# PABannier/biogpt.cpp

Measured on AMD Instinct MI355X. Metric: decode tokens/sec BioGPT Q4_0 n_ctx=1024, higher is better.
Workload: dtype int8; 1 GPU; greedy 200-token continuation of a 4-token prompt per GPU (main.cpp loop, -b 8, --top_k 1), BioGPT-base Q4_0, F32 KV cache, n_ctx=1024; 1 step = 1 continuation per rank; n_layer=24, d_model=1024, d_ff=4096, n_vocab=42384, n_predict=200, n_prompt=4, parallelism=replicas x1 (weights RCCL-broadcast once)

## Files before the change

biogpt.cpp_amd/csrc/kernels_xpipe.hip.h:

```cpp
#pragma once

#include "kernels_decode.hip.h"

namespace bgk {

typedef unsigned long long xp_u64;
typedef float xp_v4f __attribute__((ext_vector_type(4)));
#define XP_RLX __ATOMIC_RELAXED, __HIP_MEMORY_SCOPE_AGENT
constexpr uint32_t XP_SPIN_MAX = 400000u;

struct XpLayer {
    const float *ln0_w, *ln0_b, *ln1_w, *ln1_b;
    const float *bqkv, *bo, *b1, *b2;
    DevMatrix Wqkv, Wo, W1, W2;
    float *kcache, *vcache;
    unsigned long long *gx1, *gx;
};

constexpr int XP_G_QKV = 0;
constexpr int XP_G_ATT = 3072;
constexpr int XP_G_X1 = XP_G_ATT + 320;
constexpr int XP_G_H = XP_G_X1 + 1024;
constexpr int XP_G_X = XP_G_H + 1280;
constexpr int XP_G_LAYER = XP_G_X + 1024;
// ... 234 lines not shown
    for (int r = 16; r < 64; r += 16) {
        const float ov = __int_as_float(__builtin_amdgcn_readlane(__float_as_int(bv), r));
        const int oi = __builtin_amdgcn_readlane(bi, r);
        if (ov > rv || (ov == rv && oi < ri)) { rv = ov; ri = oi; }
    }
    bv = rv; bi = ri;
}
template <int WT>
__device__ __forceinline__ void xp_row4_request(const DevMatrix &m, int row, int t, uint32_t &q, uint32_t &sc, uint32_t &qh) {
    using TI = TypeInfo<WT>;
    const int64_t blk = (int64_t)row * (m.K / QK) + (t >> 3);
    const int j = (4 * t) & 31;
    if (WT == W_Q8_0) q = *reinterpret_cast<const uint32_t *>(m.qs + blk * 32 + j);
    else q = *reinterpret_cast<const uint32_t *>(m.qs + blk * 16 + (j & 15));
    sc = TI::q81 ? reinterpret_cast<const uint32_t *>(m.sc)[blk] : (uint32_t)reinterpret_cast<const uint16_t *>(m.sc)[blk];
    qh = (WT == W_Q5_0 || WT == W_Q5_1) ? m.qh[blk] : 0u;
}
template <int WT>
__device__ __forceinline__ void xp_row4_values(uint32_t q, uint32_t sc, uint32_t qh, int t, float (&e)[4]) {
    const int j = (4 * t) & 31;
#pragma unroll
    for (int i = 0; i < 4; i++) {
        if (WT == W_Q8_0) { e[i] = __fmul_rn((float)(int8_t)((q >> (8 * i)) & 0xFFu), h2f((uint16_t)sc)); continue; }
        const uint32_t byte = (q >> (8 * i)) & 0xFFu;
        int v = (j < 16) ? (int)(byte & 0x0Fu) : (int)(byte >> 4);
        if (WT == W_Q5_0 || WT == W_Q5_1) v |= (int)((qh >> (j + i)) & 1u) << 4;
        if (WT == W_Q4_0) e[i] = __fmul_rn((float)(v - 8), h2f((uint16_t)sc));
        else if (WT == W_Q5_0) e[i] = __fmul_rn((float)(v - 16), h2f((uint16_t)sc));
        else e[i] = __fadd_rn(__fmul_rn((float)v, h2f((uint16_t)(sc & 0xFFFFu))), h2f((uint16_t)(sc >> 16)));
    }
}

__device__ __forceinline__ uint32_t xp_pack4(int8_t q) {
    const int b = (int)(uint8_t)q;
    const int b1 = __builtin_amdgcn_update_dpp(0, b, 0x101, 0xf, 0xf, true);
    const int b2 = __builtin_amdgcn_update_dpp(0, b, 0x102, 0xf, 0xf, true);
    const int b3 = __builtin_amdgcn_update_dpp(0, b, 0x103, 0xf, 0xf, true);
    return (uint32_t)b | ((uint32_t)b1 << 8) | ((uint32_t)b2 << 16) | ((uint32_t)b3 << 24);
}

constexpr int XL_G_SC = 0;
constexpr int XL_G_PV = 16 * 1024;
constexpr int XL_G_LAYER = XL_G_PV + 16 * 16 * 128;

constexpr int XP_S_X = 0;
constexpr int XP_S_X1 = XP_S_X + 4096;
constexpr int XP_S_XQ = XP_S_X1 + 4096;
constexpr int XP_S_XD = XP_S_XQ + 1024;
constexpr int XP_S_XS = XP_S_XD + 128;
constexpr int XP_S_RED = XP_S_XS + 128;
constexpr int XP_S_HQ = XP_S_RED + 64;
constexpr int XP_S_HD = XP_S_HQ + 4096;
constexpr int XP_S_HS = XP_S_HD + 512;
constexpr int XP_S_PART = XP_S_HS + 512;
constexpr int XP_S_G = XP_S_PART + 256 * DEC_PS * 4;
constexpr int XP_S_LN = XP_S_G + 512;
constexpr int XP_S_BIAS = XP_S_LN + 16384;
constexpr int XP_S_CUR = XP_S_BIAS + 1536;
constexpr int XP_S_S = XP_S_CUR + 768;
constexpr int XP_S_REDF = XP_S_S + 1024;
constexpr int XP_S_REDD = XP_S_REDF + 512;
constexpr int XP_S_PV = XP_S_REDD + 128;
constexpr int XP_S_TOTAL = XP_S_PV + 8192;
static_assert(32 * DEC_PS2 <= 256 * DEC_PS, "fc2 block terms fit the shared region");
__host__ __device__ inline size_t xpipe_smem_bytes(int gelu_entries) { return XP_S_TOTAL + (size_t)gelu_entries * 2; }

template <int WT, bool EXPAND>
__device__ __forceinline__ float xp_dot(const Unit<WT> &u, const uint32_t *xq, float xd, float xs_f, int xs_i) {
    if constexpr (EXPAND) return unit_dot_settled<WT>(u, xq, xd, xs_f, xs_i);
    else return unit_dot_quant<WT>(u, xq, xd, xs_f, xs_i);
}
template <int WT, bool EXPAND>
__device__ __forceinline__ void xp_settle(Unit<WT> &u) {
    if constexpr (EXPAND) {
        settle_unit<WT>(u);
        asm volatile("" : "+v"(u.q0.x), "+v"(u.q0.y), "+v"(u.q0.z), "+v"(u.q0.w), "+v"(u.q1.x), "+v"(u.q1.y), "+v"(u.q1.z), "+v"(u.q1.w), "+v"(u.sc));
    }
}

__device__ __forceinline__ uint32_t xp_wave_sum_u32(uint32_t v) {
    int s = (int)v;
    s += dpp_i<DPP_QUAD_XOR1>(s); s += dpp_i<DPP_QUAD_XOR2>(s); s += dpp_i<DPP_ROW_HALF_MIRROR>(s); s += dpp_i<DPP_ROW_MIRROR>(s);
    return (uint32_t)((__builtin_amdgcn_readlane(s, 0) + __builtin_amdgcn_readlane(s, 16)) + (__builtin_amdgcn_readlane(s, 32) + __builtin_amdgcn_readlane(s, 48)));
}

template <int WT, int LPK, int NW, int KCAP, int ROLE, bool SPLIT, bool RES>
__device__ __forceinline__ void xp_run(const XpParams &p, unsigned char *smem, const int xcd, const int slot, const uint32_t epoch0, const int n_past0,
                                       const int n_gen0) {
    using TI = TypeInfo<WT>;
    static_assert(TI::quant && (WT != W_Q8_0 || SPLIT), "18-30 weight units per lane must fit the register file (Q8_0: 9 registers per unit: split layers)");
    static_assert(ROLE == 0 || ROLE == 1 || (ROLE == 2 && SPLIT), "0 attention head, 1 q/k/v rows, 2 (split layers) the MLP half");
    static_assert(SPLIT || TI::q81, "the producers publish Q8_0 block sums only for Q4_1 / Q5_1 (want_sum = q81): the symmetric formats need the signed units of the split form (unit_dot_settled)");
    constexpr bool ATTN = ROLE == 0;
    constexpr bool EXPAND = SPLIT;
    constexpr bool FIRST = !SPLIT || ROLE != 2, SECOND = !SPLIT || ROLE == 2;
    static_assert(LPK == 2 || LPK == 4 || LPK == 8 || LPK == 16, "lanes per key");
    static_assert(NW == 8 || NW == 16, "waves per workgroup");
    constexpr int D = 1024, DK = 64, NT = NW * 64;
    constexpr int QS = 96 / NW, OS = 16 / NW, FS = 64 / NW, F2R = 32 / NW;
    constexpr bool DUAL = SPLIT && KCAP > 256;
    constexpr int KW = DUAL ? KCAP / 2 : KCAP;
    constexpr int HI = (DUAL && ROLE == 1) ? 1 : 0;
    static_assert(KW % NW == 0 && KW <= NW * 64 / LPK, "key capacity of the launch");
    constexpr int NF4 = 16 / LPK, NV = KW / NW;
    float *const s_x = reinterpret_cast<float *>(smem + XP_S_X);
    float *const s_x1 = reinterpret_cast<float *>(smem + XP_S_X1);
    uint32_t *const s_xq = reinterpret_cast<uint32_t *>(smem + XP_S_XQ);
    float *const s_xd = reinterpret_cast<float *>(smem + XP_S_XD);
    uint32_t *const s_xs = reinterpret_cast<uint32_t *>(smem + XP_S_XS);
    double *const s_red = reinterpret_cast<double *>(smem + XP_S_RED);
    uint32_t *const s_hq = reinterpret_cast<uint32_t *>(smem + XP_S_HQ);
    float *const s_hd = reinterpret_cast<float *>(smem + XP_S_HD);
    uint32_t *const s_hs = reinterpret_cast<uint32_t *>(smem + XP_S_HS);
    float *const s_part = reinterpret_cast<float *>(smem + XP_S_PART);
    float *const s_g = reinterpret_cast<float *>(smem + XP_S_G);
    float *const s_ln = reinterpret_cast<float *>(smem + XP_S_LN);
    float *const s_bias = reinterpret_cast<float *>(smem + XP_S_BIAS);
    float *const s_cur = reinterpret_cast<float *>(smem + XP_S_CUR);
    float *const s_S = reinterpret_cast<float *>(smem + XP_S_S);
    float *const s_redf = reinterpret_cast<float *>(smem + XP_S_REDF);
    int *const s_redi = reinterpret_cast<int *>(smem + XP_S_REDF + 256);
    double *const s_redd = reinterpret_cast<double *>(smem + XP_S_REDD);
    double *const s_pv = reinterpret_cast<double *>(smem + XP_S_PV);
    uint16_t *const s_gelu = reinterpret_cast<uint16_t *>(smem + XP_S_TOTAL);
    uint32_t *const s_dead = reinterpret_cast<uint32_t *>(smem + XP_S_REDD + 96);
    uint32_t *const s_kvdead = reinterpret_cast<uint32_t *>(smem + XP_S_REDD + 64);
    uint32_t *const s_spec = reinterpret_cast<uint32_t *>(smem + XP_S_REDD + 112);
    const int t_cap = p.t_cap;
    const int n_units = SPLIT ? 2 * p.n_layer : p.n_layer;
    const int last_xcd = (n_units - 1) & 7;
    for (int tk = 0; tk < p.n_tok; tk++) {
    const uint32_t epoch = epoch0 + (uint32_t)tk;
    uint32_t etag = epoch;
    const int n_past = n_past0 + tk, T = n_past + 1;
    if (tk > 0 && __hip_atomic_load(p.ctl + 1, XP_RLX) != 0u) break;
    for (int U = xcd; U < n_units; U += 8) {
        const int L = SPLIT ? (U >> 1) : U;
        int tid = threadIdx.x;
        asm volatile("" : "+v"(tid));
        const int lane = tid & 63, wave = tid >> 6;
        const int sub = lane & 31, rsub = lane >> 5;
        const bool worker = tid < 256;
        if (tk == 0 && U == xcd && U >= 2) {
            if (tid == 0) {
                const xp_u64 *g = SPLIT ? (ROLE != 2 ? XPL(L - 1).gx1 : XPL(L - 1).gx) : XPL(L - 2).gx;
                for (uint32_t spins = 0;; spins++) {
                    if ((uint32_t)(__hip_atomic_load(g, XP_RLX) >> 32) == epoch) break;
                    if (spins >= XP_SPIN_MAX) { xp_fail(p, 3u); break; }
                    if ((spins & 255u) == 255u && __hip_atomic_load(p.ctl + 1, XP_RLX) != 0u) break;
                    __builtin_amdgcn_s_sleep(16);
                }
            }
            __syncthreads();
        }
        const XpLayerK &Y = XPL(L);
        xp_u64 *const G = p.gran + (size_t)L * XP_G_LAYER;
        constexpr bool attn_wg = ATTN || (DUAL && ROLE == 1);
        const int head = slot & 15;
        Unit<WT> wo[OS], w1[FS], w2[F2R][2];
        {
            float4 l0 = make_float4(0.f, 0.f, 0.f, 0.f), l1 = l0, l2 = l0, l3 = l0;
            if (worker) {
                if (FIRST) { l0 = xp_ldg4(Y.ln0_w, tid); l1 = xp_ldg4(Y.ln0_b, tid); }
                if (SECOND) { l2 = xp_ldg4(Y.ln1_w, tid); l3 = xp_ldg4(Y.ln1_b, tid); }
            }
            float bv = 0.0f;
// ... 117 lines not shown
                                if (XPK(spec_rec)) __hip_atomic_store(XPK(spec_rec), ((unsigned long long)want << 32) | (unsigned long long)(uint32_t)guess, __ATOMIC_RELAXED, __HIP_MEMORY_SCOPE_SYSTEM);
                                got = ahead ? guess : wait_post(want, n_past, spec);
                            }
                            if (got >= 0) {
                                xp_put_local(gt, epoch, (uint32_t)got);
                                xp_put(gt + 1, epoch, 1u);
                                s_spec[0] = (uint32_t)spec; s_spec[1] = ahead ? (uint32_t)guess : 0xffffffffu;
                            } else xp_quit(p);
                            if ((XPK(res_dbg) & 32) && XPK(wall)) XPK(wall)[(size_t)(want & 4095u) * 2] = wall_clock64();
                            if (wl4) wl4[2] = wall_clock64();
                        }
                    }
                    uint32_t v[1];
                    xp_sweep_q<RES, 1>(gt, true, epoch, v, p, etag);
                    tok = (int)v[0];
                    if (tok < 0 || tok >= XPK(n_vocab)) tok = 0;
                } else if (tk > 0) {
                    tok = sample_prev();
                    if (slot == 0 && tid == 0) {
                        int32_t *tokens = state_tokens(XPK(st));
                        const int g = n_gen0 + tk;
                        if (g < XPK(n_positions)) tokens[XPK(n_positions) + g] = tok;
                        tokens[0] = tok;
                    }
                    __syncthreads();
                } else if (XPK(tok_src) == 2) {
                    float bv = -INFINITY;
                    int bi = 0x7fffffff;
                    for (int k = tid; k < XPK(nparts); k += NT) {
                        const float v = XPK(pmax_val)[k];
                        const int ix = XPK(pmax_idx)[k];
                        if (v > bv || (v == bv && ix < bi)) { bv = v; bi = ix; }
                    }
    #pragma unroll
                    for (int off = 32; off > 0; off >>= 1) {
                        const float ov = __shfl_xor(bv, off, 64);
                        const int oi = __shfl_xor(bi, off, 64);
                        if (ov > bv || (ov == bv && oi < bi)) { bv = ov; bi = oi; }
                    }
                    if (lane == 0) { s_redf[wave] = bv; s_redi[wave] = bi; }
                    __syncthreads();
                    bv = s_redf[0]; bi = s_redi[0];
    #pragma unroll
                    for (int w = 1; w < NW; w++)
                        if (s_redf[w] > bv || (s_redf[w] == bv && s_redi[w] < bi)) { bv = s_redf[w]; bi = s_redi[w]; }
                    tok = bi;
                    if (tok < 0 || tok >= XPK(n_vocab)) tok = 0;
                    if (slot == 0 && tid == 0) {
                        int32_t *tokens = state_tokens(XPK(st));
                        const int g = n_gen0;
                        if (g < XPK(n_positions)) tokens[XPK(n_positions) + g] = tok;
                        tokens[0] = tok;
                    }
                } else {
                    tok = (RES && p.resident != 0) ? XPK(res_tok0) : state_tokens(XPK(st))[0];
                }
                if (slot == 0) XP_TAIL(tk, 5);
                if (worker) {
                    float e[4];
                    if (emb_fast) {
                        uint32_t tq, tsc, tqh;
                        xp_row4_request<WT>(XPK_MATRIX(tok_emb), tok, tid, tq, tsc, tqh);
                        float te[4], pe[4];
                        xp_row4_values<WT>(pq, psc, pqh, tid, pe);
                        xp_row4_values<WT>(tq, tsc, tqh, tid, te);
    #pragma unroll
                        for (int j = 0; j < 4; j++) e[j] = __fadd_rn(__fmul_rn(te[j], XPK(embed_scale)), pe[j]);
                    } else {
    #pragma unroll
                        for (int j = 0; j < 4; j++)
                            e[j] = __fadd_rn(__fmul_rn(dequant_elem(XPK_MATRIX(tok_emb), tok, 4 * tid + j), XPK(embed_scale)), dequant_elem(XPK_MATRIX(pos_emb), n_past + 2, 4 * tid + j));
                    }
                    xv = make_float4(e[0], e[1], e[2], e[3]);
                }
            } else if (wave < 4) {
                uint32_t v[4];
                xp_sweep_q<RES, 4, 256, true>(XPL(L - 1).gx + tid, true, epoch, v, p, etag);
                xv = make_float4(__uint_as_float(v[0]), __uint_as_float(v[1]), __uint_as_float(v[2]), __uint_as_float(v[3]));
            }
            if (RES && wave < 4 && lane == 0) { s_dead[wave] = (etag == 0u) ? 1u : 0u; }
            return xv;
        };
        if constexpr (FIRST) {
        constexpr bool MERGE = SPLIT && KCAP <= 128;
        if (!attn_wg && MERGE) {
            const float4 xv = layer_input();
            if (worker) reinterpret_cast<float4 *>(s_x)[tid] = xv;
            XP_WALL(0);
        }
        if (!attn_wg && !MERGE) {
            constexpr int Q0 = (KCAP <= 192) ? QS / 3 : 0;
            Unit<WT> wqkv[QS];
#pragma unroll
            for (int s = Q0; s < QS; s++) {
                const int jj = s * 2 * NW + wave * 2 + rsub;
                load_unit<WT>(wqkv[s], XPL_MATRIX(Y.Wqkv), (int64_t)((jj >> 6) * 1024 + head * 64 + (jj & 63)) * 32 + sub);
            }
#pragma unroll
            for (int s = Q0; s < QS; s++) xp_settle<WT, EXPAND>(wqkv[s]);
            const float4 xv = layer_input();
            XP_WALL(0);
            float4 lnw = xv, lnb = xv;
            if (worker) {
                reinterpret_cast<float4 *>(s_x)[tid] = xv;
                lnw = reinterpret_cast<const float4 *>(s_ln)[tid]; lnb = reinterpret_cast<const float4 *>(s_ln + 1024)[tid];
            }
            ln4_q8_1024<TI::q81, TI::q81>(xv, lnw, lnb, p.eps, s_red, s_xq, s_xd, s_xs);
            XP_WALL(6);
            uint32_t ax[8];
            const uint4 a = *reinterpret_cast<const uint4 *>(s_xq + sub * 8), b = *reinterpret_cast<const uint4 *>(s_xq + sub * 8 + 4);
            ax[0] = a.x; ax[1] = a.y; ax[2] = a.z; ax[3] = a.w; ax[4] = b.x; ax[5] = b.y; ax[6] = b.z; ax[7] = b.w;
            const float axd = s_xd[sub];
            const uint32_t axs = s_xs[sub];
            float *const part = s_part + wave * 2 * QS * DEC_PS;
#pragma unroll
            for (int s = Q0; s < QS; s++) part[(s * 2 + rsub) * DEC_PS + sub] = xp_dot<WT, EXPAND>(wqkv[s], ax, axd, __uint_as_float(axs), (int)axs);
            __builtin_amdgcn_fence(__ATOMIC_RELEASE, "wavefront");
            __builtin_amdgcn_wave_barrier();
            __builtin_amdgcn_fence(__ATOMIC_ACQUIRE, "wavefront");
            if (lane >= 2 * Q0 && lane < 2 * QS) {
                const int jj = (lane >> 1) * 2 * NW + wave * 2 + (lane & 1);
                float v = __fadd_rn(s_bias[jj], sum32_in_order(part + lane * DEC_PS));
                const int which = jj >> 6, d = jj & 63;
                if (which == 0) v = __fmul_rn(v, p.q_scale);
                xp_put_local(G + XP_G_QKV + which * 1024 + head * 64 + d, etag, __float_as_uint(v));
                if (which != 0 && (!RES || (etag != 0u && (s_dead[0] | s_dead[1] | s_dead[2] | s_dead[3]) == 0u))) {
                    float *kc_ = Y.kcache, *vc_ = Y.vcache;
                    asm volatile("" : "+s"(kc_), "+s"(vc_));
                    ((__attribute__((address_space(1))) float *)((which == 1) ? kc_ : vc_))[((size_t)head * p.P + n_past) * DK + d] = v;
                }
            }
            XP_WALL(1);
        }
        if (attn_wg) {
            float4 kr[NF4];
            float vr[NV];
            const int ksub = tid & (LPK - 1), kidx = tid / LPK;
            const int dd = tid & (DK - 1), sl = tid >> 6;
            {
                constexpr bool KV_SC1 = !MERGE;
                const float *kb = Y.kcache + (size_t)head * p.P * DK, *vb = Y.vcache + (size_t)head * p.P * DK;
                const __amdgpu_buffer_rsrc_t krs = xp_kv_rsrc(kb, p.P * DK * 4), vrs = xp_kv_rsrc(vb, p.P * DK * 4);
                if (KV_SC1 || kidx < t_cap) {
#pragma unroll
                    for (int m = 0; m < NF4; m++) kr[m] = xp_kv_load4<KV_SC1>(krs, kb, ((HI * KW + kidx) * (DK / 4) + ksub + LPK * m) * 4);
                } else {
#pragma unroll
                    for (int m = 0; m < NF4; m++) kr[m] = make_float4(0.f, 0.f, 0.f, 0.f);
                }
#pragma unroll
                for (int k = 0; k < NV; k++) {
                    const int j = HI * KW + sl + NW * k;
                    vr[k] = (KV_SC1 || j < t_cap) ? xp_kv_load1<KV_SC1>(vrs, vb, j * DK + dd) : 0.0f;
                }
            }
            if constexpr (MERGE) {
                Unit<WT> wqkv[QS];
#pragma unroll
                for (int s = 0; s < QS; s++) {
                    const int jj = s * 2 * NW + wave * 2 + rsub;
                    load_unit<WT>(wqkv[s], XPL_MATRIX(Y.Wqkv), (int64_t)((jj >> 6) * 1024 + head * 64 + (jj & 63)) * 32 + sub);
                }
#pragma unroll
                for (int s = 0; s < QS; s++) xp_settle<WT, EXPAND>(wqkv[s]);
                const float4 xv = layer_input();
                XP_WALL(0);
                if (L == 0 && slot == 0) { asm volatile("" :: "v"(xv.x)); XP_TAIL(tk, 6); }
                float4 lnw = xv, lnb = xv;
                if (worker) {
                    reinterpret_cast<float4 *>(s_x)[tid] = xv;
                    lnw = reinterpret_cast<const float4 *>(s_ln)[tid]; lnb = reinterpret_cast<const float4 *>(s_ln + 1024)[tid];
                }
                ln4_q8_1024<TI::q81, TI::q81>(xv, lnw, lnb, p.eps, s_red, s_xq, s_xd, s_xs);
                XP_WALL(6);
                if (L == 0 && slot == 0) XP_TAIL(tk, 7);
                uint32_t ax[8];
                const uint4 a = *reinterpret_cast<const uint4 *>(s_xq + sub * 8), b = *reinterpret_cast<const uint4 *>(s_xq + sub * 8 + 4);
                ax[0] = a.x; ax[1] = a.y; ax[2] = a.z; ax[3] = a.w; ax[4] = b.x; ax[5] = b.y; ax[6] = b.z; ax[7] = b.w;
                const float axd = s_xd[sub];
                const uint32_t axs = s_xs[sub];
                float *const part = s_part + wave * 2 * QS * DEC_PS;
#pragma unroll
                for (int s = 0; s < QS; s++) part[(s * 2 + rsub) * DEC_PS + sub] = xp_dot<WT, EXPAND>(wqkv[s], ax, axd, __uint_as_float(axs), (int)axs);
                __builtin_amdgcn_fence(__ATOMIC_RELEASE, "wavefront");
                __builtin_amdgcn_wave_barrier();
                __builtin_amdgcn_fence(__ATOMIC_ACQUIRE, "wavefront");
                if (lane < 2 * QS) {
                    const int jj = (lane >> 1) * 2 * NW + wave * 2 + (lane & 1);
                    float v = __fadd_rn(s_bias[jj], sum32_in_order(part + lane * DEC_PS));
                    const int which = jj >> 6, d = jj & 63;
                    if (which == 0) v = __fmul_rn(v, p.q_scale);
                    s_cur[jj] = v;
                    if (which != 0 && (!RES || (etag != 0u && (s_dead[0] | s_dead[1] | s_dead[2] | s_dead[3]) == 0u))) {
                        float *kc_ = Y.kcache, *vc_ = Y.vcache;
                        asm volatile("" : "+s"(kc_), "+s"(vc_));
                        ((__attribute__((address_space(1))) float *)((which == 1) ? kc_ : vc_))[((size_t)head * p.P + n_past) * DK + d] = v;
                    }
                }
                XP_WALL(1);
            } else if constexpr (DUAL) {
                constexpr int QH = QS / 2;
                Unit<WT> wq[QH];
#pragma unroll
                for (int s = 0; s < QH; s++) {
                    const int jj = (HI * QH + s) * 2 * NW + wave * 2 + rsub;
                    load_unit<WT>(wq[s], XPL_MATRIX(Y.Wqkv), (int64_t)((jj >> 6) * 1024 + head * 64 + (jj & 63)) * 32 + sub);
                }
#pragma unroll
                for (int s = 0; s < QH; s++) xp_settle<WT, EXPAND>(wq[s]);
                const float4 xv = layer_input();
                XP_WALL(0);
                float4 lnw = xv, lnb = xv;
                if (worker) {
                    reinterpret_cast<float4 *>(s_x)[tid] = xv;
                    lnw = reinterpret_cast<const float4 *>(s_ln)[tid]; lnb = reinterpret_cast<const float4 *>(s_ln + 1024)[tid];
                }
                ln4_q8_1024<TI::q81, TI::q81>(xv, lnw, lnb, p.eps, s_red, s_xq, s_xd, s_xs);
                XP_WALL(6);
                uint32_t ax[8];
                const uint4 a = *reinterpret_cast<const uint4 *>(s_xq + sub * 8), b = *reinterpret_cast<const uint4 *>(s_xq + sub * 8 + 4);
                ax[0] = a.x; ax[1] = a.y; ax[2] = a.z; ax[3] = a.w; ax[4] = b.x; ax[5] = b.y; ax[6] = b.z; ax[7] = b.w;
                const float axd = s_xd[sub];
                const uint32_t axs = s_xs[sub];
                float *const part = s_part + wave * 2 * QH * DEC_PS;
#pragma unroll
                for (int s = 0; s < QH; s++) part[(s * 2 + rsub) * DEC_PS + sub] = xp_dot<WT, EXPAND>(wq[s], ax, axd, __uint_as_float(axs), (int)axs);
                __builtin_amdgcn_fence(__ATOMIC_RELEASE, "wavefront");
                __builtin_amdgcn_wave_barrier();
                __builtin_amdgcn_fence(__ATOMIC_ACQUIRE, "wavefront");
                if (lane < 2 * QH) {
                    const int jj = (HI * QH + (lane >> 1)) * 2 * NW + wave * 2 + (lane & 1);
                    float v = __fadd_rn(s_bias[jj], sum32_in_order(part + lane * DEC_PS));
                    const int which = jj >> 6, d = jj & 63;
                    if (which == 0) v = __fmul_rn(v, p.q_scale);
                    s_cur[jj] = v;
                    xp_put_local(G + XP_G_QKV + which * 1024 + head * 64 + d, etag, __float_as_uint(v));
                    if (which != 0 && (!RES || (etag != 0u && (s_dead[0] | s_dead[1] | s_dead[2] | s_dead[3]) == 0u))) {
                        float *kc_ = Y.kcache, *vc_ = Y.vcache;
                        asm volatile("" : "+s"(kc_), "+s"(vc_));
                        ((__attribute__((address_space(1))) float *)((which == 1) ? kc_ : vc_))[((size_t)head * p.P + n_past) * DK + d] = v;
                    }
                }
                XP_WALL(1);
                if (wave < 2) {
                    uint32_t v[1];
                    const int jo = (1 - HI) * 96 + (tid < 96 ? tid : 0);
                    xp_sweep_q<RES, 1>(G + XP_G_QKV + (jo >> 6) * 1024 + head * 64 + (jo & 63), tid < 96, epoch, v, p, etag);
                    if (tid < 96) s_cur[jo] = __uint_as_float(v[0]);
                    if (RES && lane == 0) { s_kvdead[wave] = (etag == 0u) ? 1u : 0u; }
                }
            } else if constexpr (KCAP <= 192) {
                constexpr int Q0 = QS / 3;
                Unit<WT> wq[Q0];
#pragma unroll
                for (int s = 0; s < Q0; s++) {
                    const int jj = s * 2 * NW + wave * 2 + rsub;
                    load_unit<WT>(wq[s], XPL_MATRIX(Y.Wqkv), (int64_t)(head * 64 + jj) * 32 + sub);
                }
#pragma unroll
                for (int s = 0; s < Q0; s++) xp_settle<WT, EXPAND>(wq[s]);
                const float4 xv = layer_input();
                XP_WALL(0);
                float4 lnw = xv, lnb = xv;
                if (worker) {
                    reinterpret_cast<float4 *>(s_x)[tid] = xv;
                    lnw = reinterpret_cast<const float4 *>(s_ln)[tid]; lnb = reinterpret_cast<const float4 *>(s_ln + 1024)[tid];
                }
                ln4_q8_1024<TI::q81, TI::q81>(xv, lnw, lnb, p.eps, s_red, s_xq, s_xd, s_xs);
                XP_WALL(6);
                uint32_t ax[8];
                const uint4 a = *reinterpret_cast<const uint4 *>(s_xq + sub * 8), b = *reinterpret_cast<const uint4 *>(s_xq + sub * 8 + 4);
                ax[0] = a.x; ax[1] = a.y; ax[2] = a.z; ax[3] = a.w; ax[4] = b.x; ax[5] = b.y; ax[6] = b.z; ax[7] = b.w;
                const float axd = s_xd[sub];
                const uint32_t axs = s_xs[sub];
                float *const part = s_part + wave * 2 * Q0 * DEC_PS;
#pragma unroll
                for (int s = 0; s < Q0; s++) part[(s * 2 + rsub) * DEC_PS + sub] = xp_dot<WT, EXPAND>(wq[s], ax, axd, __uint_as_float(axs), (int)axs);
                __builtin_amdgcn_fence(__ATOMIC_RELEASE, "wavefront");
                __builtin_amdgcn_wave_barrier();
                __builtin_amdgcn_fence(__ATOMIC_ACQUIRE, "wavefront");
                if (lane < 2 * Q0) {
                    const int jj = (lane >> 1) * 2 * NW + wave * 2 + (lane & 1);
                    s_cur[jj] = __fmul_rn(__fadd_rn(s_bias[jj], sum32_in_order(part + lane * DEC_PS)), p.q_scale);
                }
                XP_WALL(1);
            } else {
                {
                    const float4 xv = layer_input();
                    if (worker) reinterpret_cast<float4 *>(s_x)[tid] = xv;
                }
                XP_WALL(0);
                if (wave < 3) {
                    uint32_t v[1];
                    xp_sweep_q<RES, 1>(G + XP_G_QKV + wave * 1024 + head * 64 + lane, true, epoch, v, p, etag);
                    s_cur[tid] = __uint_as_float(v[0]);
                }
            }
            __syncthreads();
            if constexpr (RES && DUAL) { if ((s_kvdead[0] | s_kvdead[1]) != 0u) etag = 0u; }
            XP_WALL(7);
            constexpr bool LATE_KV = !MERGE && KCAP <= 192;
            auto key_score = [&](const float4 (&kk)[NF4]) __attribute__((always_inline)) -> float {
                double a0 = 0.0, a1 = 0.0, a2 = 0.0, a3 = 0.0;
#pragma unroll
                for (int m = 0; m < NF4; m++) {
                    const float4 qm = *reinterpret_cast<const float4 *>(s_cur + 4 * (LPK * m + ksub));
                    a0 += (double)__fmul_rn(kk[m].x, qm.x); a1 += (double)__fmul_rn(kk[m].y, qm.y);
                    a2 += (double)__fmul_rn(kk[m].z, qm.z); a3 += (double)__fmul_rn(kk[m].w, qm.w);
                }
                double acc = (a0 + a1) + (a2 + a3);
                acc += dpp_d<DPP_QUAD_XOR1>(acc);
                if (LPK >= 4) acc += dpp_d<DPP_QUAD_XOR2>(acc);
                if (LPK >= 8) acc += dpp_d<DPP_ROW_HALF_MIRROR>(acc);
                if (LPK >= 16) acc += dpp_d<DPP_ROW_MIRROR>(acc);
                return (float)acc;
            };
            if constexpr (LATE_KV) {
                if (wave >= NW - 2) {
                    uint32_t v[1];
                    const int which = wave - (NW - 3);
                    xp_sweep_q<RES, 1>(G + XP_G_QKV + which * 1024 + head * 64 + lane, true, epoch, v, p, etag);
                    s_cur[which * 64 + lane] = __uint_as_float(v[0]);
                    if (RES && lane == 0) { s_kvdead[which - 1] = (etag == 0u) ? 1u : 0u; }
                }
            }
            float sc = -INFINITY;
            const int jg = HI * KW + kidx;
            if (HI * KW * LPK + (tid & ~63) < LPK * T) {
                if (!LATE_KV && jg == n_past) {
#pragma unroll
                    for (int m = 0; m < NF4; m++) kr[m] = *reinterpret_cast<const float4 *>(s_cur + 64 + 4 * (LPK * m + ksub));
                }
                if (jg < T && !(LATE_KV && jg == n_past)) sc = key_score(kr);
            }
            static_assert(NW == 8, "key j = wave + 8 k sits in lane (wave + 8 k) & 63 of slot k >> 3");
            constexpr bool SMW = KCAP <= 64;
            constexpr int KC = (KCAP + 63) / 64;
            [[maybe_unused]] float ev[KC];
            float inv;
            if constexpr (SMW) {
                if (ksub == 0) s_S[kidx] = sc;
                __syncthreads();
                float scl[KC];
#pragma unroll
                for (int c = 0; c < KC; c++) scl[c] = s_S[lane + 64 * c];
                if constexpr (LATE_KV) {
                    if (RES && (s_kvdead[0] | s_kvdead[1]) != 0u) etag = 0u;
                    float4 kn[NF4];
#pragma unroll
                    for (int m = 0; m < NF4; m++) kn[m] = *reinterpret_cast<const float4 *>(s_cur + 64 + 4 * (LPK * m + ksub));
                    const float snew = key_score(kn);
#pragma unroll
                    for (int c = 0; c < KC; c++) if (lane + 64 * c == n_past) scl[c] = snew;
                }
                float mx = scl[0];
#pragma unroll
                for (int c = 1; c < KC; c++) mx = fmaxf(mx, scl[c]);
                mx = wave_max_f32(mx);
                XP_WALL(13);
                uint32_t ulo = 0u, uhi = 0u;
#pragma unroll
                for (int c = 0; c < KC; c++) {
                    float val = 0.0f;
                    if (lane + 64 * c < T) {
                        const uint32_t ix = f2h(__fsub_rn(scl[c], mx)), neg = ix - 0x8000u;
                        uint16_t e16;
                        if (neg < (uint32_t)p.exp_n) e16 = s_gelu[neg];
                        else if (p.exp_n > 0 && ix == 0u) e16 = 0x3C00;
                        else if (p.exp_n > 0 && neg < 0x7C00u) e16 = 0;
                        else e16 = p.exp_tab[ix];
                        val = h2f(e16);
                    }
                    ev[c] = val;
                    const uint32_t u = (uint32_t)__fmul_rn(val, 16777216.0f);
                    ulo += u & 0xFFFFu; uhi += u >> 16;
                }
                ulo = xp_wave_sum_u32(ulo); uhi = xp_wave_sum_u32(uhi);
                const double sum = ((double)uhi * 65536.0 + (double)ulo) * 0x1p-24;
                inv = inv_sum_f32(sum);
            } else {
                if constexpr (LATE_KV) {
                    __syncthreads();
                    if (RES && (s_kvdead[0] | s_kvdead[1]) != 0u) etag = 0u;
                    if (kidx == n_past) {
#pragma unroll
                        for (int m = 0; m < NF4; m++) kr[m] = *reinterpret_cast<const float4 *>(s_cur + 64 + 4 * (LPK * m + ksub));
                        sc = key_score(kr);
                    }
                }
                bool valid = jg < T && ksub == 0;
                if constexpr (DUAL) {
                    static_assert(LPK == 2, "two lanes per key: the second one takes the partner's score of the same index");
                    xp_u64 *const gsc = p.gran_l + (size_t)L * XL_G_LAYER + XL_G_SC + head * 1024;
                    if (valid) xp_put_local(gsc + jg, etag, __float_as_uint(sc));
                    const int jo = (1 - HI) * KW + kidx;
                    const bool theirs = ksub == 1 && jo < T;
                    uint32_t v[1];
                    xp_sweep_q<RES, 1>(gsc + jo, theirs, epoch, v, p, etag);
                    if (theirs) { sc = __uint_as_float(v[0]); valid = true; }
                }
                float mx = wave_max_f32(sc);
                if (lane == 0) s_redf[wave] = mx;
                if (RES && DUAL && lane == 0) reinterpret_cast<uint32_t *>(s_redf)[NW + wave] = (etag == 0u) ? 1u : 0u;
                __syncthreads();
                mx = s_redf[0];
#pragma unroll
                for (int w = 1; w < NW; w++) mx = fmaxf(mx, s_redf[w]);
                if constexpr (RES && DUAL) {
                    uint32_t dead = 0u;
#pragma unroll
                    for (int w = 0; w < NW; w++) dead |= reinterpret_cast<const uint32_t *>(s_redf)[NW + w];
                    if ((dead) != 0u) etag = 0u;
                }
                XP_WALL(13);
                double sum = 0.0;
                if (valid) {
                    const uint32_t ix = f2h(__fsub_rn(sc, mx)), neg = ix - 0x8000u;
                    uint16_t e16;
                    if (neg < (uint32_t)p.exp_n) e16 = s_gelu[neg];
                    else if (p.exp_n > 0 && ix == 0u) e16 = 0x3C00;
                    else if (p.exp_n > 0 && neg < 0x7C00u) e16 = 0;
                    else e16 = p.exp_tab[ix];
                    const float val = h2f(e16);
                    if (ksub == 0) s_S[kidx] = val;
                    sum = (double)val;
                }
                sum = wave_sum_f64(sum);
                if (lane == 0) s_redd[wave] = sum;
                __syncthreads();
                sum = 0.0;
#pragma unroll
                for (int w = 0; w < NW; w++) sum += s_redd[w];
                inv = inv_sum_f32(sum);
            }
            XP_WALL(14);
            {
                const float vcur = s_cur[128 + dd];
                [[maybe_unused]] const int wave_u = __builtin_amdgcn_readfirstlane(wave);
                constexpr int CH = NV < 16 ? NV : (NV % 16 == 0 ? 16 : 8);
                double a0 = 0.0, a1 = 0.0;
#pragma unroll
                for (int k0 = 0; k0 < NV; k0 += CH) {
                    float pj[CH];
#pragma unroll
                    for (int k = 0; k < CH; k++) {
                        if constexpr (SMW) pj[k] = __int_as_float(__builtin_amdgcn_readlane(__float_as_int(ev[(k0 + k) >> 3]), wave_u + 8 * ((k0 + k) & 7)));
                        else pj[k] = s_S[sl + NW * (k0 + k)];
                    }
#pragma unroll
                    for (int k = 0; k < CH; k += 2) {
                        const int j0 = HI * KW + sl + NW * (k0 + k), j1 = j0 + NW;
                        const double c0 = (double)__fmul_rn(j0 == n_past ? vcur : vr[k0 + k], __fmul_rn(pj[k], inv));
                        const double c1 = (double)__fmul_rn(j1 == n_past ? vcur : vr[k0 + k + 1], __fmul_rn(pj[k + 1], inv));
                        a0 += (j0 < T) ? c0 : 0.0;
                        a1 += (j1 < T) ? c1 : 0.0;
                    }
                }
                s_pv[tid] = a0 + a1;
            }
            __syncthreads();
            XP_WALL(15);
            if (tid < DK) {
                double t0 = 0.0, t1 = 0.0;
#pragma unroll
                for (int s2 = 0; s2 < NW; s2 += 2) { t0 += s_pv[s2 * DK + tid]; t1 += s_pv[(s2 + 1) * DK + tid]; }
                double tot = t0 + t1;
                [[maybe_unused]] xp_u64 *const gpv = DUAL ? p.gran_l + (size_t)L * XL_G_LAYER + XL_G_PV + head * 16 * 128 : nullptr;
                if constexpr (DUAL && HI == 1) {
                    xp_put_local(gpv + tid, etag, (uint32_t)__double2loint(tot)); xp_put_local(gpv + 64 + tid, etag, (uint32_t)__double2hiint(tot));
                } else {
                    if constexpr (DUAL) {
                        uint32_t v[2];
                        xp_sweep_q<RES, 2, 64>(gpv + tid, true, epoch, v, p, etag);
                        tot += __hiloint2double((int)v[1], (int)v[0]);
                    }
                    const float o = (float)tot;
                    int8_t q8; float d8; uint32_t s8;
                    q8_block32(o, TI::q81, q8, d8, s8, TI::q81);
                    const uint32_t packed = xp_pack4(q8);
                    const int blk = head * 2 + (tid >> 5);
                    if ((tid & 3) == 0) xp_put_local(G + XP_G_ATT + head * 16 + (tid >> 2), etag, packed);
                    if ((tid & 31) == 0) { xp_put_local(G + XP_G_ATT + 256 + blk, etag, __float_as_uint(d8)); if (TI::q81) xp_put_local(G + XP_G_ATT + 288 + blk, etag, s8); }
                }
            }
        }
        XP_WALL(2);
        if (wave < 5) {
// ... 371 lines not shown
```

Measured before the change: 4167 tokens/s.

## Let attention workgroup own q/k rows per KV bucket, fetch v late

Replaces the MERGE/LATE_KV split with a per-KV-capacity ownership count (OWN = 0, 2 or 3 row groups) that says how many of the head's q/k/v row groups the attention workgroup computes itself. With OWN=2 in the 129-256 buckets, the attention workgroup now computes q and k locally and appends k to the cache. Only v is fetched from the producer, via an early relaxed atomic load with a fallback sweep, and it is written to the cache after the scores. This removes the late-key score patching and its extra barrier, and moves part of the QKV GEMV onto the attention workgroup. The cost is more register pressure and longer critical-path work in that workgroup.

```diff
diff --git a/biogpt.cpp_amd/csrc/kernels_xpipe.hip.h b/biogpt.cpp_amd/csrc/kernels_xpipe.hip.h
--- a/biogpt.cpp_amd/csrc/kernels_xpipe.hip.h
+++ b/biogpt.cpp_amd/csrc/kernels_xpipe.hip.h
@@ -340,6 +340,26 @@
     int s = (int)v;
     s += dpp_i<DPP_QUAD_XOR1>(s); s += dpp_i<DPP_QUAD_XOR2>(s); s += dpp_i<DPP_ROW_HALF_MIRROR>(s); s += dpp_i<DPP_ROW_MIRROR>(s);
     return (uint32_t)((__builtin_amdgcn_readlane(s, 0) + __builtin_amdgcn_readlane(s, 16)) + (__builtin_amdgcn_readlane(s, 32) + __builtin_amdgcn_readlane(s, 48)));
+}
+
+template <int WT, int KCAP, bool RES>
+constexpr int xp_own() {
+#ifdef XP_OWN_64
+    if (KCAP <= 64) return XP_OWN_64;
+#endif
+#ifdef XP_OWN_128
+    if (KCAP > 64 && KCAP <= 128) return XP_OWN_128;
+#endif
+#ifdef XP_OWN_192
+    if (KCAP > 128 && KCAP <= 192) return XP_OWN_192;
+#endif
+#ifdef XP_OWN_256
+    if (KCAP > 192 && KCAP <= 256) return XP_OWN_256;
+#endif
+    if (KCAP <= 128) return 3;
+    if (KCAP <= 192) return 2;
+    if (WT == W_Q8_0) return 0;
+    return 2;
 }
 
 template <int WT, int LPK, int NW, int KCAP, int ROLE, bool SPLIT, bool RES>
@@ -623,14 +643,17 @@
             return xv;
         };
         if constexpr (FIRST) {
-        constexpr bool MERGE = SPLIT && KCAP <= 128;
-        if (!attn_wg && MERGE) {
+        constexpr int OWN = (DUAL || !SPLIT) ? 0 : xp_own<WT, KCAP, RES>();
+        static_assert(OWN == 0 || OWN == 2 || OWN == 3, "row groups of the head's own workgroup (1 -- k and v late, behind the old keys' scores -- lost in every bucket and is gone)");
+        constexpr int NOWN = OWN * QS / 3;
+        constexpr bool K_HOME = OWN >= 2, V_HOME = OWN >= 2;
+        if (!attn_wg && OWN == 3) {
             const float4 xv = layer_input();
             if (worker) reinterpret_cast<float4 *>(s_x)[tid] = xv;
             XP_WALL(0);
         }
-        if (!attn_wg && !MERGE) {
-            constexpr int Q0 = (KCAP <= 192) ? QS / 3 : 0;
+        if (!attn_wg && OWN < 3) {
+            constexpr int Q0 = NOWN;
             Unit<WT> wqkv[QS];
 #pragma unroll
             for (int s = Q0; s < QS; s++) {
@@ -665,7 +688,8 @@
                 const int which = jj >> 6, d = jj & 63;
                 if (which == 0) v = __fmul_rn(v, p.q_scale);
                 xp_put_local(G + XP_G_QKV + which * 1024 + head * 64 + d, etag, __float_as_uint(v));
-                if (which != 0 && (!RES || (etag != 0u && (s_dead[0] | s_dead[1] | s_dead[2] | s_dead[3]) == 0u))) {
+                const bool appends = which == 1 ? !K_HOME : (which == 2 && !V_HOME);
+                if (appends && (!RES || (etag != 0u && (s_dead[0] | s_dead[1] | s_dead[2] | s_dead[3]) == 0u))) {
                     float *kc_ = Y.kcache, *vc_ = Y.vcache;
                     asm volatile("" : "+s"(kc_), "+s"(vc_));
                     ((__attribute__((address_space(1))) float *)((which == 1) ? kc_ : vc_))[((size_t)head * p.P + n_past) * DK + d] = v;
@@ -679,12 +703,12 @@
             const int ksub = tid & (LPK - 1), kidx = tid / LPK;
             const int dd = tid & (DK - 1), sl = tid >> 6;
             {
-                constexpr bool KV_SC1 = !MERGE;
+                constexpr bool K_SC1 = DUAL || !K_HOME, V_SC1 = DUAL || !V_HOME;
                 const float *kb = Y.kcache + (size_t)head * p.P * DK, *vb = Y.vcache + (size_t)head * p.P * DK;
                 const __amdgpu_buffer_rsrc_t krs = xp_kv_rsrc(kb, p.P * DK * 4), vrs = xp_kv_rsrc(vb, p.P * DK * 4);
-                if (KV_SC1 || kidx < t_cap) {
-#pragma unroll
-                    for (int m = 0; m < NF4; m++) kr[m] = xp_kv_load4<KV_SC1>(krs, kb, ((HI * KW + kidx) * (DK / 4) + ksub + LPK * m) * 4);
+                if (K_SC1 || kidx < t_cap) {
+#pragma unroll
+                    for (int m = 0; m < NF4; m++) kr[m] = xp_kv_load4<K_SC1>(krs, kb, ((HI * KW + kidx) * (DK / 4) + ksub + LPK * m) * 4);
                 } else {
 #pragma unroll
                     for (int m = 0; m < NF4; m++) kr[m] = make_float4(0.f, 0.f, 0.f, 0.f);
@@ -692,18 +716,18 @@
 #pragma unroll
                 for (int k = 0; k < NV; k++) {
                     const int j = HI * KW + sl + NW * k;
-                    vr[k] = (KV_SC1 || j < t_cap) ? xp_kv_load1<KV_SC1>(vrs, vb, j * DK + dd) : 0.0f;
-                }
-            }
-            if constexpr (MERGE) {
-                Unit<WT> wqkv[QS];
-#pragma unroll
-                for (int s = 0; s < QS; s++) {
+                    vr[k] = (V_SC1 || j < t_cap) ? xp_kv_load1<V_SC1>(vrs, vb, j * DK + dd) : 0.0f;
+                }
+            }
+            if constexpr (!DUAL && NOWN > 0) {
+                Unit<WT> wqkv[NOWN];
+#pragma unroll
+                for (int s = 0; s < NOWN; s++) {
                     const int jj = s * 2 * NW + wave * 2 + rsub;
                     load_unit<WT>(wqkv[s], XPL_MATRIX(Y.Wqkv), (int64_t)((jj >> 6) * 1024 + head * 64 + (jj & 63)) * 32 + sub);
                 }
 #pragma unroll
-                for (int s = 0; s < QS; s++) xp_settle<WT, EXPAND>(wqkv[s]);
+                for (int s = 0; s < NOWN; s++) xp_settle<WT, EXPAND>(wqkv[s]);
                 const float4 xv = layer_input();
                 XP_WALL(0);
                 if (L == 0 && slot == 0) { asm volatile("" :: "v"(xv.x)); XP_TAIL(tk, 6); }
@@ -720,19 +744,19 @@
                 ax[0] = a.x; ax[1] = a.y; ax[2] = a.z; ax[3] = a.w; ax[4] = b.x; ax[5] = b.y; ax[6] = b.z; ax[7] = b.w;
                 const float axd = s_xd[sub];
                 const uint32_t axs = s_xs[sub];
-                float *const part = s_part + wave * 2 * QS * DEC_PS;
-#pragma unroll
-                for (int s = 0; s < QS; s++) part[(s * 2 + rsub) * DEC_PS + sub] = xp_dot<WT, EXPAND>(wqkv[s], ax, axd, __uint_as_float(axs), (int)axs);
+                float *const part = s_part + wave * 2 * NOWN * DEC_PS;
+#pragma unroll
+                for (int s = 0; s < NOWN; s++) part[(s * 2 + rsub) * DEC_PS + sub] = xp_dot<WT, EXPAND>(wqkv[s], ax, axd, __uint_as_float(axs), (int)axs);
                 __builtin_amdgcn_fence(__ATOMIC_RELEASE, "wavefront");
                 __builtin_amdgcn_wave_barrier();
                 __builtin_amdgcn_fence(__ATOMIC_ACQUIRE, "wavefront");
-                if (lane < 2 * QS) {
+                if (lane < 2 * NOWN) {
                     const int jj = (lane >> 1) * 2 * NW + wave * 2 + (lane & 1);
                     float v = __fadd_rn(s_bias[jj], sum32_in_order(part + lane * DEC_PS));
                     const int which = jj >> 6, d = jj & 63;
                     if (which == 0) v = __fmul_rn(v, p.q_scale);
                     s_cur[jj] = v;
-                    if (which != 0 && (!RES || (etag != 0u && (s_dead[0] | s_dead[1] | s_dead[2] | s_dead[3]) == 0u))) {
+                    if (OWN >= 2 && which != 0 && (!RES || (etag != 0u && (s_dead[0] | s_dead[1] | s_dead[2] | s_dead[3]) == 0u))) {
                         float *kc_ = Y.kcache, *vc_ = Y.vcache;
                         asm volatile("" : "+s"(kc_), "+s"(vc_));
                         ((__attribute__((address_space(1))) float *)((which == 1) ? kc_ : vc_))[((size_t)head * p.P + n_past) * DK + d] = v;
@@ -790,41 +814,6 @@
                     if (tid < 96) s_cur[jo] = __uint_as_float(v[0]);
                     if (RES && lane == 0) { s_kvdead[wave] = (etag == 0u) ? 1u : 0u; }
                 }
-            } else if constexpr (KCAP <= 192) {
-                constexpr int Q0 = QS / 3;
-                Unit<WT> wq[Q0];
-#pragma unroll
-                for (int s = 0; s < Q0; s++) {
-                    const int jj = s * 2 * NW + wave * 2 + rsub;
-                    load_unit<WT>(wq[s], XPL_MATRIX(Y.Wqkv), (int64_t)(head * 64 + jj) * 32 + sub);
-                }
-#pragma unroll
-                for (int s = 0; s < Q0; s++) xp_settle<WT, EXPAND>(wq[s]);
-                const float4 xv = layer_input();
-                XP_WALL(0);
-                float4 lnw = xv, lnb = xv;
-                if (worker) {
-                    reinterpret_cast<float4 *>(s_x)[tid] = xv;
-                    lnw = reinterpret_cast<const float4 *>(s_ln)[tid]; lnb = reinterpret_cast<const float4 *>(s_ln + 1024)[tid];
-                }
-                ln4_q8_1024<TI::q81, TI::q81>(xv, lnw, lnb, p.eps, s_red, s_xq, s_xd, s_xs);
-                XP_WALL(6);
-                uint32_t ax[8];
-                const uint4 a = *reinterpret_cast<const uint4 *>(s_xq + sub * 8), b = *reinterpret_cast<const uint4 *>(s_xq + sub * 8 + 4);
-                ax[0] = a.x; ax[1] = a.y; ax[2] = a.z; ax[3] = a.w; ax[4] = b.x; ax[5] = b.y; ax[6] = b.z; ax[7] = b.w;
-                const float axd = s_xd[sub];
-                const uint32_t axs = s_xs[sub];
-                float *const part = s_part + wave * 2 * Q0 * DEC_PS;
-#pragma unroll
-                for (int s = 0; s < Q0; s++) part[(s * 2 + rsub) * DEC_PS + sub] = xp_dot<WT, EXPAND>(wq[s], ax, axd, __uint_as_float(axs), (int)axs);
-                __builtin_amdgcn_fence(__ATOMIC_RELEASE, "wavefront");
-                __builtin_amdgcn_wave_barrier();
-                __builtin_amdgcn_fence(__ATOMIC_ACQUIRE, "wavefront");
-                if (lane < 2 * Q0) {
-                    const int jj = (lane >> 1) * 2 * NW + wave * 2 + (lane & 1);
-                    s_cur[jj] = __fmul_rn(__fadd_rn(s_bias[jj], sum32_in_order(part + lane * DEC_PS)), p.q_scale);
-                }
-                XP_WALL(1);
             } else {
                 {
                     const float4 xv = layer_input();
@@ -840,7 +829,7 @@
             __syncthreads();
             if constexpr (RES && DUAL) { if ((s_kvdead[0] | s_kvdead[1]) != 0u) etag = 0u; }
             XP_WALL(7);
-            constexpr bool LATE_KV = !MERGE && KCAP <= 192;
+            constexpr bool LATE_V = !DUAL && OWN == 2;
             auto key_score = [&](const float4 (&kk)[NF4]) __attribute__((always_inline)) -> float {
                 double a0 = 0.0, a1 = 0.0, a2 = 0.0, a3 = 0.0;
 #pragma unroll
@@ -856,23 +845,28 @@
                 if (LPK >= 16) acc += dpp_d<DPP_ROW_MIRROR>(acc);
                 return (float)acc;
             };
-            if constexpr (LATE_KV) {
-                if (wave >= NW - 2) {
-                    uint32_t v[1];
-                    const int which = wave - (NW - 3);
-                    xp_sweep_q<RES, 1>(G + XP_G_QKV + which * 1024 + head * 64 + lane, true, epoch, v, p, etag);
-                    s_cur[which * 64 + lane] = __uint_as_float(v[0]);
-                    if (RES && lane == 0) { s_kvdead[which - 1] = (etag == 0u) ? 1u : 0u; }
-                }
+            [[maybe_unused]] xp_u64 v_first = 0ull;
+            if constexpr (LATE_V) {
+                if (wave == NW - 1 && (!RES || etag != 0u)) v_first = __hip_atomic_load((xp_gq)(G + XP_G_QKV + 2 * 1024 + head * 64 + lane), XP_RLX);
             }
             float sc = -INFINITY;
             const int jg = HI * KW + kidx;
             if (HI * KW * LPK + (tid & ~63) < LPK * T) {
-                if (!LATE_KV && jg == n_past) {
+                if (jg == n_past) {
 #pragma unroll
                     for (int m = 0; m < NF4; m++) kr[m] = *reinterpret_cast<const float4 *>(s_cur + 64 + 4 * (LPK * m + ksub));
                 }
-                if (jg < T && !(LATE_KV && jg == n_past)) sc = key_score(kr);
+                if (jg < T) sc = key_score(kr);
+            }
+            if constexpr (LATE_V) {
+                if (wave == NW - 1) {
+                    uint32_t v[1] = {(uint32_t)v_first};
+                    if (!__all((uint32_t)(v_first >> 32) == epoch)) xp_sweep_q<RES, 1>(G + XP_G_QKV + 2 * 1024 + head * 64 + lane, true, epoch, v, p, etag);
+                    s_cur[128 + lane] = __uint_as_float(v[0]);
+                    if (!RES || (etag != 0u && (s_dead[0] | s_dead[1] | s_dead[2] | s_dead[3]) == 0u))
+                        ((__attribute__((address_space(1))) float *)Y.vcache)[((size_t)head * p.P + n_past) * DK + lane] = __uint_as_float(v[0]);
+                    if (RES && lane == 0) { s_kvdead[1] = (etag == 0u) ? 1u : 0u; }
+                }
             }
             static_assert(NW == 8, "key j = wave + 8 k sits in lane (wave + 8 k) & 63 of slot k >> 3");
             constexpr bool SMW = KCAP <= 64;
@@ -885,15 +879,7 @@
                 float scl[KC];
 #pragma unroll
                 for (int c = 0; c < KC; c++) scl[c] = s_S[lane + 64 * c];
-                if constexpr (LATE_KV) {
-                    if (RES && (s_kvdead[0] | s_kvdead[1]) != 0u) etag = 0u;
-                    float4 kn[NF4];
-#pragma unroll
-                    for (int m = 0; m < NF4; m++) kn[m] = *reinterpret_cast<const float4 *>(s_cur + 64 + 4 * (LPK * m + ksub));
-                    const float snew = key_score(kn);
-#pragma unroll
-                    for (int c = 0; c < KC; c++) if (lane + 64 * c == n_past) scl[c] = snew;
-                }
+                if constexpr (RES && LATE_V) { if (s_kvdead[1] != 0u) etag = 0u; }
                 float mx = scl[0];
 #pragma unroll
                 for (int c = 1; c < KC; c++) mx = fmaxf(mx, scl[c]);
@@ -920,15 +906,6 @@
                 const double sum = ((double)uhi * 65536.0 + (double)ulo) * 0x1p-24;
                 inv = inv_sum_f32(sum);
             } else {
-                if constexpr (LATE_KV) {
-                    __syncthreads();
-                    if (RES && (s_kvdead[0] | s_kvdead[1]) != 0u) etag = 0u;
-                    if (kidx == n_past) {
-#pragma unroll
-                        for (int m = 0; m < NF4; m++) kr[m] = *reinterpret_cast<const float4 *>(s_cur + 64 + 4 * (LPK * m + ksub));
-                        sc = key_score(kr);
-                    }
-                }
                 bool valid = jg < T && ksub == 0;
                 if constexpr (DUAL) {
                     static_assert(LPK == 2, "two lanes per key: the second one takes the partner's score of the same index");
@@ -944,6 +921,7 @@
                 if (lane == 0) s_redf[wave] = mx;
                 if (RES && DUAL && lane == 0) reinterpret_cast<uint32_t *>(s_redf)[NW + wave] = (etag == 0u) ? 1u : 0u;
                 __syncthreads();
+                if constexpr (RES && LATE_V) { if (s_kvdead[1] != 0u) etag = 0u; }
                 mx = s_redf[0];
 #pragma unroll
                 for (int w = 1; w < NW; w++) mx = fmaxf(mx, s_redf[w]);
```

After: 4164 tokens/s. Within noise of the previous version (-0.1%).
